# facebookresearch/sam-audio

Hardware: AMD Instinct MI355X
Metric: seconds-of-audio separated/sec/node (higher is better)
Workload: dtype fp16x3 (fp32 storage as the reference; every big contraction on IEEE-half hi + lo split operands: 3 MFMA products per multiply, fp32 accumulation - fp32-grade results on the 16-bit matrix cores)

## Files before the change

### sam_audio_amd/csrc/api.hip

```cpp
#include <cstring>
#include <string>

#include "engine.h"
#include "peav.h"

struct samaudio_ctx {
  sa::Engine* engine;
};
struct samaudio_judge {
  sa::Judge* judge;
};
struct samaudio_frame {
  sa::FramePredictor* frame;
};

namespace {
thread_local std::string g_err;
}
namespace sa {
void set_last_error(const std::string& msg) { g_err = msg; }
}
namespace {
int ret(const sa::Status& s) {
  if (!s.ok()) g_err = s.msg;
// ... 153 lines not shown
    out[n].ms = k.ms;
    ++n;
  }
  *count = n;
  return SAMAUDIO_OK;
}

int samaudio_op_gemm(const void* params_host, size_t params_bytes, int precision, samaudio_stream stream) {
  if (!params_host || params_bytes != sizeof(sa::GemmParams)) return bad("samaudio_op_gemm: GemmParams size mismatch");
  sa::GemmParams p;
  std::memcpy(&p, params_host, sizeof(p));
  const bool bf16 = precision == SAMAUDIO_BF16;
  if (const char* why = sa::gemm_check(p, bf16)) return bad(why);
  return hip_ret(sa::launch_gemm(p, bf16, (hipStream_t)stream), "gemm");
}

int samaudio_op_resunit(const void* conv7_params_host, const void* conv1_params_host, size_t params_bytes,
                        samaudio_stream stream) {
  if (!conv7_params_host || !conv1_params_host || params_bytes != sizeof(sa::GemmParams))
    return bad("samaudio_op_resunit: GemmParams size mismatch");
  sa::GemmParams p, q;
  std::memcpy(&p, conv7_params_host, sizeof(p));
  std::memcpy(&q, conv1_params_host, sizeof(q));
  if (const char* why = sa::gemm_check(p, true)) return bad(why);
  if (const char* why = sa::gemm_check(q, true)) return bad(why);
  if (!sa::resunit_ok(p, q)) return bad("samaudio_op_resunit: not a (k7, k1) residual-unit pair the fused kernel covers");
  return hip_ret(sa::launch_resunit(p, q, (hipStream_t)stream), "resunit");
}

int samaudio_op_rmsnorm_mod(const float* x, const float* w, const float* shift_tab, const float* scale_tab,
                            const float* tvec, int64_t tvec_ld, int shift_off, int scale_off, void* out,
                            int precision, int rows, int dim, int rows_per_batch, float eps, samaudio_stream stream) {
  if (dim % 4) return bad("rmsnorm_mod: dim % 4");
  return hip_ret(sa::launch_rmsnorm_mod(x, w, shift_tab, scale_tab, tvec, tvec_ld, shift_off, scale_off, out,
                                        precision == SAMAUDIO_BF16, rows, dim, rows_per_batch, eps,
                                        (hipStream_t)stream), "rmsnorm_mod");
}

int samaudio_op_groupnorm_silu(const float* x, const float* w, const float* b, void* partials_f64, void* out,
                               int precision, int batch, int frames, int channels, int halo, float eps,
                               samaudio_stream stream) {
  if (channels % 4) return bad("groupnorm: channels % 4");
  return hip_ret(sa::launch_groupnorm_silu(x, w, b, (double*)partials_f64, out, precision == SAMAUDIO_BF16, batch,
                                           frames, channels, halo, eps, (hipStream_t)stream), "groupnorm_silu");
}

int samaudio_op_qkv_prep(const void* qkv, const float* q_w, const float* k_w, const float* rope_cos,
                         const float* rope_sin, void* q, void* k, void* vt, int precision, int batch, int frames,
// ... 262 lines not shown
```

### sam_audio_amd/csrc/engine.hip

```cpp
#include "engine.h"

#include <algorithm>
#include <cmath>
#include <cstdio>
#include <cstdlib>
#include <cstring>

namespace sa {

#define SA_TRY(expr)                     \
  do {                                   \
    Status _s = (expr);                  \
    if (!_s.ok()) return _s;             \
  } while (0)
#define SA_HIP(expr)                                                                  \
  do {                                                                                \
    hipError_t _e = (expr);                                                           \
    if (_e != hipSuccess)                                                             \
      return Status{SAMAUDIO_ERR_HIP, std::string(#expr) + ": " + hipGetErrorString(_e)}; \
  } while (0)

static Status fail(int code, const std::string& m) { return Status{code, m}; }

static bool trace_on() {
// ... 752 lines not shown
  p.out_act = nullptr; p.act_ld = p.act_bstride = p.act_off = 0; p.act = ACT_NONE; p.f32_act = 0;
  const double flops = alg_flops >= 0 ? alg_flops : 2.0 * p_in.M * (double)p_in.N * p_in.K * p_in.nbatch;
  SA_TRY(gemm(p, st, flops, SAMAUDIO_CLS_CODEC, p_in.K == c && p_in.kc == c ? GemmKind::X3 : GemmKind::X3Block));
  if (!p_in.out_act || (act == ACT_NONE && !p_in.out_f32)) return Status{};
  const long start = p_in.c_ld_rel ? p_in.c_lo : 0, count = p_in.c_ld_rel ? p_in.c_hi - p_in.c_lo : (long)p_in.M * p_in.N;
  const int chan = p_in.chan_mod ? p_in.chan_mod : p_in.N;
  if (start % chan) return fail(SAMAUDIO_ERR_ARG, "gemm_codec_x3: window start is not a whole channel row");
  return op("codec_act", (double)count * p_in.nbatch * 8, 0, st, [&] {
    return launch_act_flat(raw + raw_off + start, raw_bs, (float*)p_in.out_act + p_in.act_off + start, p_in.act_bstride, p_in.nbatch, count,
                           chan, act, p_in.act_alpha, st);
  });
}

Status Engine::res_unit(GemmParams p, GemmParams q, void*& cur, void*& alt, double flops7, double flops1, hipStream_t st) {
  p.out_act = alt;
  q.A = alt;
  q.out_act = cur;
  GemmParams fp = p, fq = q;
  fq.out_act = alt;
  fp.tag = fq.tag = phase_ == Phase::Codec ? 1 : 0;
  const bool covered = p.N == 64 || p.N == 96 || p.N == 128 || p.N == 192;
  const bool fuse = bf16_ && covered && !debug_flag(DBG_RESUNIT_TWO_LAUNCHES) && resunit_ok(fp, fq) &&
                    ((long)((p.M + 255) / 256) * p.nbatch >= 256 || debug_flag(DBG_RESUNIT_FUSE_ALWAYS));
  if (!fuse) {
    SA_TRY(codec_gemm(p, st, flops7));
    return codec_gemm(q, st, flops1);
  }
  if (const char* why = gemm_check(fp, bf16_)) return fail(SAMAUDIO_ERR_ARG, why);
  if (const char* why = gemm_check(fq, bf16_)) return fail(SAMAUDIO_ERR_ARG, why);
  const double inter = (double)p.M * p.N * p.nbatch * esz_;
  SA_TRY(op("resunit_bf16", gemm_alg_bytes(fp, esz_) + gemm_alg_bytes(fq, esz_) - 2 * inter, flops7 + flops1, st,
            [&] { return launch_resunit(fp, fq, st); }));
  SA_TRY(scan_out(fq, SAMAUDIO_CLS_CODEC, GemmKind::Native, st));
  std::swap(cur, alt);
  return Status{};
}

template <class F>
Status Engine::op(const char* name, double alg_bytes, double alg_flops, hipStream_t st, F&& launch) {
  if (!prof_on_) {
    SA_HIP(launch());
    return Status{};
  }
  ProfRec r;
  r.key = std::string(phase_name()) + "/" + name;
  r.flops = alg_flops;
// ... 759 lines not shown
```

### sam_audio_amd/csrc/gemm.hip

```cpp
#include "common.h"
#include "kernels.h"

#include <type_traits>

namespace sa {

typedef h16x8_t bf16x8_t;
typedef __attribute__((ext_vector_type(4))) float f32x4_t;

template <typename T> struct Mma;
template <> struct Mma<bf16_t> {
  typedef bf16x8_t frag_t;
  static __device__ __forceinline__ f32x4_t run(const frag_t& a, const frag_t& b, f32x4_t c) {
    return SA_MFMA_16x16x32(a, b, c);
  }
};
template <> struct Mma<float> {
  typedef f32x4_t frag_t;
  static __device__ __forceinline__ f32x4_t run(const frag_t& a, const frag_t& b, f32x4_t c) {
    c = __builtin_amdgcn_mfma_f32_16x16x4f32(a[0], b[0], c, 0, 0, 0);
    c = __builtin_amdgcn_mfma_f32_16x16x4f32(a[1], b[1], c, 0, 0, 0);
    c = __builtin_amdgcn_mfma_f32_16x16x4f32(a[2], b[2], c, 0, 0, 0);
    c = __builtin_amdgcn_mfma_f32_16x16x4f32(a[3], b[3], c, 0, 0, 0);
    return c;
  }
};

__device__ __forceinline__ float quant16(float x, int fmt) {
  if (fmt == GEMM_QUANT_BF16) {
    unsigned u = __float_as_uint(x);
    u += 0x7fffu + ((u >> 16) & 1u);
    return __uint_as_float(u & 0xffff0000u);
  }
  if (fmt == GEMM_QUANT_FP16) return (float)(_Float16)x;
  return x;
}
__device__ __forceinline__ f32x4_t quant16x4(f32x4_t v, int fmt) {
  return f32x4_t{quant16(v[0], fmt), quant16(v[1], fmt), quant16(v[2], fmt), quant16(v[3], fmt)};
}

__device__ __forceinline__ void dma16(const void* gsrc, char* lds_wave_base) {
  __builtin_amdgcn_global_load_lds((const __attribute__((address_space(1))) void*)gsrc,
                                   (__attribute__((address_space(3))) void*)lds_wave_base, 16, 0, 0);
}

template <typename T, int BM, int BN, int WM_, int WN_, bool FLY = false>
__global__ __launch_bounds__(256, (FLY ? 2 : 1)) void gemm_kernel(const GemmParams p) {
  constexpr int NW = WM_ * WN_;
  static_assert(NW == 4, "4 waves per workgroup");
  constexpr int CH = 16 / (int)sizeof(T);
  constexpr int BK = 128 / (int)sizeof(T);
  constexpr int WTM = BM / WM_, WTN = BN / WN_;
  constexpr int FM = WTM / 16, FN = WTN / 16;
  constexpr int AI = BM / 32, BI = BN / 32;
  static_assert(BM % 32 == 0 && BN % 32 == 0 && WTM % 16 == 0 && WTN % 16 == 0, "tile shape");
  constexpr int TILE_A = BM * 128, TILE_B = BN * 128, STAGE = TILE_A + TILE_B;
  constexpr int NS = 2;
  __shared__ __attribute__((aligned(16))) char smem[NS * STAGE];

  const int tid = threadIdx.x;
  const int lane = tid & 63;
  const int wave = __builtin_amdgcn_readfirstlane(tid >> 6);
  const int wm = wave / WN_, wn = wave % WN_;

  const int tiles_n = (p.N + BN - 1) / BN;
  const int tiles_m = (p.M + BM - 1) / BM;
  int id = blockIdx.x;
  const int tn = id % tiles_n;
  id /= tiles_n;
  const int tm = id % tiles_m;
// ... 28 lines not shown
    char* sA = smem + stage * STAGE;
    char* sB = sA + TILE_A;
#pragma unroll
    for (int i = 0; i < AI; ++i) dma16(a_rows[i] + a_tap + a_in, sA + (wave + 4 * i) * 1024);
#pragma unroll
    for (int i = 0; i < BI; ++i) dma16(w_rows[i], sB + (wave + 4 * i) * 1024);
    a_in += BK;
    while (a_in >= p.kc) { a_in -= p.kc; a_tap += p.tap_stride; }
#pragma unroll
    for (int i = 0; i < BI; ++i) w_rows[i] += BK;
  };

  f32x4_t acc[FM][FN];
#pragma unroll
  for (int i = 0; i < FM; ++i)
#pragma unroll
    for (int j = 0; j < FN; ++j) acc[i][j] = f32x4_t{0.f, 0.f, 0.f, 0.f};

  const int nslab = p.K / BK;
  const int lr = lane & 15, lg = lane >> 4;
  const int qa = gemm_quant_a(p.flags), qw = gemm_quant_w(p.flags);
  const bool x3fly = FLY || (sizeof(T) == 4 && (p.flags & GEMM_FLAG_X3_FLY) != 0);
  const bool wfly = FLY || (p.flags & GEMM_FLAG_W_FLY16) != 0;
  auto fly_slab = [&](const char* sA, const char* sB) {
#pragma clang fp contract(off)
        bf16x8_t ah[FM], al[FM], bh[FN], bl[FN];
        auto cl = [](float x) { return __builtin_amdgcn_fmed3f(x, -kH16Max, kH16Max); };
        auto split = [&](const char* base, int row, bf16x8_t& hi, bf16x8_t& lo) {
          const int sw = (row >> 1) & 7;
          const f32x4_t v0 = *(const f32x4_t*)(base + row * 128 + ((lg ^ sw) << 4));
          const f32x4_t v1 = *(const f32x4_t*)(base + row * 128 + (((4 + lg) ^ sw) << 4));
          unsigned h[4], l[4];
          h[0] = pack_h16x2(cl(v0[0]), cl(v0[1]));
          h[1] = pack_h16x2(cl(v0[2]), cl(v0[3]));
          h[2] = pack_h16x2(cl(v1[0]), cl(v1[1]));
          h[3] = pack_h16x2(cl(v1[2]), cl(v1[3]));
          l[0] = pack_h16x2(v0[0] - h16_lo(h[0]), v0[1] - h16_hi(h[0]));
          l[1] = pack_h16x2(v0[2] - h16_lo(h[1]), v0[3] - h16_hi(h[1]));
          l[2] = pack_h16x2(v1[0] - h16_lo(h[2]), v1[1] - h16_hi(h[2]));
          l[3] = pack_h16x2(v1[2] - h16_lo(h[3]), v1[3] - h16_hi(h[3]));
          typedef __attribute__((ext_vector_type(4))) unsigned u32x4_t;
          hi = __builtin_bit_cast(bf16x8_t, (u32x4_t){h[0], h[1], h[2], h[3]});
          lo = __builtin_bit_cast(bf16x8_t, (u32x4_t){l[0], l[1], l[2], l[3]});
        };
        if (wfly) {
#pragma unroll
          for (int j = 0; j < FN; ++j) {
            const int row = wn * WTN + j * 16 + lr, sw = (row >> 1) & 7;
            bh[j] = *(const bf16x8_t*)(sB + row * 128 + ((lg ^ sw) << 4));
            bl[j] = *(const bf16x8_t*)(sB + row * 128 + (((4 + lg) ^ sw) << 4));
          }
        } else {
#pragma unroll
          for (int j = 0; j < FN; ++j) split(sB, wn * WTN + j * 16 + lr, bh[j], bl[j]);
        }
#pragma unroll
        for (int i = 0; i < FM; ++i) split(sA, wm * WTM + i * 16 + lr, ah[i], al[i]);
#pragma unroll
        for (int i = 0; i < FM; ++i)
#pragma unroll
          for (int j = 0; j < FN; ++j) acc[i][j] = SA_MFMA_16x16x32(bh[j], al[i], acc[i][j]);
#pragma unroll
        for (int i = 0; i < FM; ++i)
#pragma unroll
          for (int j = 0; j < FN; ++j) acc[i][j] = SA_MFMA_16x16x32(bl[j], ah[i], acc[i][j]);
#pragma unroll
// ... 27 lines not shown
#pragma unroll
      for (int j = 0; j < FN; ++j) {
        const int row = wn * WTN + j * 16 + lr;
        bfr[j] = *(const typename Mma<T>::frag_t*)(sB + row * 128 + ((c ^ ((row >> 1) & 7)) << 4));
      }
      if constexpr (sizeof(T) == 4) {
        if (qa) {
#pragma unroll
          for (int i = 0; i < FM; ++i) af[i] = quant16x4(af[i], qa);
        }
        if (qw) {
#pragma unroll
          for (int j = 0; j < FN; ++j) bfr[j] = quant16x4(bfr[j], qw);
        }
      }
#pragma unroll
      for (int i = 0; i < FM; ++i)
#pragma unroll
        for (int j = 0; j < FN; ++j) acc[i][j] = Mma<T>::run(bfr[j], af[i], acc[i][j]);
    }
    }
  }

  const long bM = (long)b * p.M;
  const int n_out = p.swiglu ? p.N >> 1 : p.N;
  auto finish = [&](float v, const float bias, const float gate, const float res, const float sa, float& a) -> float {
    v += bias;
    if (p.gate) v *= gate;
    v *= p.alpha;
    v += res;
    a = v;
    if (p.act == ACT_SNAKE) a = snake_f(v, sa);
    else if (p.act == ACT_TANH) a = tanhf(v);
    else if (p.act == ACT_SILU) a = silu_f(v);
    else if (p.act == ACT_GELU) a = gelu_f(v);
    else if (p.act == ACT_QUICK_GELU) a = quick_gelu_f(v);
    else if (p.act == ACT_RELU) a = relu_f(v);
    else if (p.act == ACT_GELU_TANH) a = gelu_tanh_f(v);
    return v;
  };
  if constexpr (sizeof(T) == 4) {
    auto al16 = [](const void* q, long a, long b2, long c) { return (((size_t)q) & 15) == 0 && !((a | b2 | c) & 3); };
    const bool lean = !p.swiglu && !p.gate && !p.chan_mod && !p.c_ld_rel && !(p.N & 3) && (!p.bias || al16(p.bias, 0, 0, 0)) &&
                      (p.act != ACT_SNAKE || al16(p.act_alpha, 0, 0, 0)) && (!p.res || al16(p.res, p.res_off, p.res_ld, p.res_bstride)) &&
                      (!p.out_f32 || al16(p.out_f32, p.f32_off, p.f32_ld, p.f32_bstride)) &&
                      (!p.out_act || al16(p.out_act, p.act_off, p.act_ld, p.act_bstride));
    if (lean && (p.act == ACT_NONE || p.act == ACT_SNAKE)) {
      constexpr int CPR = BN / 4, RPI = 64 / CPR, WR = BM / 4, NIT = (WR + RPI - 1) / RPI;
      static_assert(BN % 32 == 0 && BM * BN * 4 <= NS * STAGE, "epilogue staging area");
      __syncthreads();
#pragma unroll
      for (int i = 0; i < FM; ++i)
#pragma unroll
        for (int j = 0; j < FN; ++j) {
          const int row = wm * WTM + i * 16 + lr, c = wn * (WTN / 4) + j * 4 + lg;
          *(f32x4_t*)(smem + row * (BN * 4) + ((c ^ (row & 7)) << 4)) = acc[i][j];
        }
      __syncthreads();
      const float4 z = make_float4(0.f, 0.f, 0.f, 0.f);
      const int c = lane % CPR, rsub = lane / CPR;
      const bool lane_on = rsub < RPI;
      const int n = n0 + c * 4;
      const int ncl = n < p.N ? n : p.N - 4;
      const float4 bb = p.bias ? *(const float4*)(p.bias + ncl) : z;
      const float4 sa = p.act == ACT_SNAKE ? *(const float4*)(p.act_alpha + ncl) : z;
      const float* const res0 = p.res ? p.res + p.res_off + (long)b * p.res_bstride + ncl : nullptr;
      float* const f320 = p.out_f32 ? p.out_f32 + p.f32_off + (long)b * p.f32_bstride + n : nullptr;
      float* const act0 = p.out_act ? (float*)p.out_act + p.act_off + (long)b * p.act_bstride + n : nullptr;
      const int rw = wave * WR;
      auto body = [&](auto SNAKE) {
        auto fin = [&](float v, const float bias, const float res, const float sal, float& a) -> float {
          v += bias;
          v *= p.alpha;
          v += res;
          a = decltype(SNAKE)::value ? snake_f(v, sal) : v;
          return v;
        };
        auto res_of = [&](int it) {
          const int m = m0 + rw + it * RPI + rsub;
          return res0 ? *(const float4*)(res0 + (long)(m < p.M ? m : p.M - 1) * p.res_ld) : z;
        };
        float4 rr = res_of(0);
#pragma unroll 1
        for (int it = 0; it < NIT; ++it) {
          const float4 rn = it + 1 < NIT ? res_of(it + 1) : z;
          const int rl = it * RPI + rsub, row = rw + (rl < WR ? rl : 0), m = m0 + row;
          const float4 sv = *(const float4*)(smem + row * (BN * 4) + ((c ^ (row & 7)) << 4));
          float a0, a1, a2, a3;
          const float v0 = fin(sv.x, bb.x, rr.x, sa.x, a0), v1 = fin(sv.y, bb.y, rr.y, sa.y, a1), v2 = fin(sv.z, bb.z, rr.z, sa.z, a2),
                      v3 = fin(sv.w, bb.w, rr.w, sa.w, a3);
          if (lane_on && rl < WR && m < p.M && n < p.N) {
            if (f320) *(float4*)(f320 + (long)m * p.f32_ld) = p.f32_act ? make_float4(a0, a1, a2, a3) : make_float4(v0, v1, v2, v3);
            if (act0) *(float4*)(act0 + (long)m * p.act_ld) = make_float4(a0, a1, a2, a3);
          }
          rr = rn;
        }
      };
      if (p.act == ACT_SNAKE) body(std::true_type{});
      else body(std::false_type{});
      return;
    }
  }
#pragma unroll
  for (int i = 0; i < FM; ++i) {
    const int m = m0 + wm * WTM + i * 16 + lr;
    if (m >= p.M) continue;
    const float* grow = nullptr;
    if (p.gate) grow = p.gate + ((bM + m) / p.rows_per_gate) * p.gate_ld;
    const float* rrow = p.res ? p.res + p.res_off + (long)b * p.res_bstride + (long)m * p.res_ld : nullptr;
    float* frow = p.out_f32 ? p.out_f32 + p.f32_off + (long)b * p.f32_bstride + (long)m * p.f32_ld : nullptr;
    T* arow = p.out_act ? (T*)p.out_act + p.act_off + (long)b * p.act_bstride + (long)m * p.act_ld : nullptr;
#pragma unroll
    for (int j = 0; j < FN; ++j) {
      if (p.swiglu && (j & 1)) continue;
      f32x4_t v4 = acc[i][j];
      int n = n0 + wn * WTN + j * 16 + lg * 4;
      if (p.swiglu) {
        const f32x4_t g = acc[i][j | 1];
#pragma unroll
        for (int e = 0; e < 4; ++e) v4[e] = silu_f(v4[e]) * g[e];
        n = ((n0 + wn * WTN) >> 1) + (j >> 1) * 16 + lg * 4;
      }
      if (n >= n_out) continue;
      size_t al = 0;
      if (p.bias) al |= (size_t)(p.bias + n);
      if (grow) al |= (size_t)(grow + n);
      if (p.gate_tab) al |= (size_t)(p.gate_tab + n);
      if (rrow) al |= (size_t)(rrow + n);
      if (p.act == ACT_SNAKE) al |= (size_t)(p.act_alpha + n);
      if (frow) al |= (size_t)(frow + n);
      if (arow) al |= (size_t)(arow + n) * (16 / (4 * sizeof(T)));
      if (n + 4 <= n_out && !p.chan_mod && !p.c_ld_rel && (al & 15) == 0) {
        const float4 z = make_float4(0.f, 0.f, 0.f, 0.f);
        const float4 bb = p.bias ? *(const float4*)(p.bias + n) : z;
        float4 gg = grow ? *(const float4*)(grow + n) : z;
        if (grow && p.gate_tab) { const float4 tt = *(const float4*)(p.gate_tab + n); gg.x += tt.x; gg.y += tt.y; gg.z += tt.z; gg.w += tt.w; }
        const float4 rr = rrow ? *(const float4*)(rrow + n) : z;
        const float4 sa = p.act == ACT_SNAKE ? *(const float4*)(p.act_alpha + n) : z;
        float a0, a1, a2, a3;
        const float v0 = finish(v4[0], bb.x, gg.x, rr.x, sa.x, a0), v1 = finish(v4[1], bb.y, gg.y, rr.y, sa.y, a1),
                    v2 = finish(v4[2], bb.z, gg.z, rr.z, sa.z, a2), v3 = finish(v4[3], bb.w, gg.w, rr.w, sa.w, a3);
        if (frow) *(float4*)(frow + n) = p.f32_act ? make_float4(a0, a1, a2, a3) : make_float4(v0, v1, v2, v3);
        if (arow) store4<T>(arow + n, a0, a1, a2, a3);
        continue;
      }
#pragma unroll
      for (int e = 0; e < 4; ++e) {
        const int ne = n + e;
        if (ne >= n_out) continue;
        const int ch = p.chan_mod ? ne % p.chan_mod : ne;
        const long erel = (long)m * p.c_ld_rel + ne;
        if (p.c_ld_rel && (erel < p.c_lo || erel >= p.c_hi)) continue;
        float a;
        const float v = finish(v4[e], p.bias ? p.bias[ch] : 0.f, grow ? (p.gate_tab ? p.gate_tab[ne] : 0.f) + grow[ne] : 0.f,
                               rrow ? rrow[ne] : 0.f, p.act == ACT_SNAKE ? p.act_alpha[ch] : 0.f, a);
        if (frow) frow[ne] = p.f32_act ? a : v;
        if (arow) Elem<T>::store(arow + ne, a);
      }
    }
  }
}

template <typename T, int BM, int BN, int WM_, int WN_>
static hipError_t launch_cfg(const GemmParams& p, hipStream_t st) {
  const long tiles = (long)((p.M + BM - 1) / BM) * ((p.N + BN - 1) / BN) * p.nbatch;
  hipLaunchKernelGGL((gemm_kernel<T, BM, BN, WM_, WN_>), dim3((unsigned)tiles), dim3(256), 0, st, p);
  return hipGetLastError();
}

static int g_force = -1;
void gemm_force_variant(int v) { g_force = v; }

const char* gemm_variant_name(int v, bool is_bf16) {
  const GemmVariantRow* r = gemm_variant_row(v);
  return !r ? "" : is_bf16 ? r->name16 : r->name32;
}

static GemmVariant gemm1_variant(const GemmParams& p) {
  const int N = p.N;
  if (p.swiglu) return GV_GEMM_128x128;
  if (N <= 32 || N == 96) return GV_GEMM_128x32;
  if (N <= 64 || (N % 128 != 0 && N % 64 == 0 && N <= 448)) return GV_GEMM_128x64;
  const long t128 = (long)((p.M + 127) / 128) * ((N + 127) / 128) * p.nbatch;
// ... 54 lines not shown
}

hipError_t launch_gemm(const GemmParams& p, bool is_bf16, hipStream_t st) {
  if (const int full = gemm_tail_split(p, is_bf16)) {
    const hipError_t e = launch_gemm8_split(p, full, 0, st);
    return e != hipSuccess ? e : launch_gemm8_split(p, full, 1, st);
  }
  const int v = gemm_variant(p, is_bf16);
  if (v >= GV_FLY_128x96) {
    const auto go = [&](auto kern, int bm, int bn) {
      const long tiles = (long)((p.M + bm - 1) / bm) * ((p.N + bn - 1) / bn) * p.nbatch;
      hipLaunchKernelGGL(kern, dim3((unsigned)tiles), dim3(256), 0, st, p);
      return hipGetLastError();
    };
    switch (v) {
      case GV_FLY_128x96: return go(gemm_kernel<float, 128, 96, 4, 1, true>, 128, 96);
      case GV_FLY_128x128: return go(gemm_kernel<float, 128, 128, 4, 1, true>, 128, 128);
      case GV_FLY_128x64: return go(gemm_kernel<float, 128, 64, 4, 1, true>, 128, 64);
      default: return go(gemm_kernel<float, 128, 32, 4, 1, true>, 128, 32);
    }
  }
  if (v > GV_GEMM_128x32) return launch_gemm2(p, (GemmVariant)v, st);
  return is_bf16 ? launch_t<bf16_t>(p, v, st) : launch_t<float>(p, v, st);
}

static const char* need_8phase(const GemmParams& p, bool is_bf16, bool (*eligible)(const GemmParams&), const char* not_eligible,
                               const char* not_chosen) {
  if (!is_bf16 || !gemm2_ok(p) || !eligible(p)) return not_eligible;
  return gemm_is_8phase(gemm_variant(p, is_bf16)) ? nullptr : not_chosen;
}
const char* gemm_check(const GemmParams& p, bool is_bf16) {
  const int bk = is_bf16 ? 64 : 32, ch = is_bf16 ? 8 : 4;
  if (p.M <= 0 || p.N <= 0 || p.K <= 0 || p.nbatch <= 0) return "gemm: empty problem";
  if (p.K % bk) return "gemm: K must be a multiple of 64 (bf16) / 32 (f32) - pad W with zeros";
  if (p.kc % ch || p.kc <= 0) return "gemm: kc must be a positive multiple of the 16-byte chunk";
  if ((p.lda % ch) || (p.tap_stride % ch) || (p.a_off % ch) || (p.a_bstride % ch))
    return "gemm: A strides/offsets must be 16-byte aligned";
  if (p.swiglu && (p.N % 32)) return "gemm: swiglu needs N % 32 == 0";
  if (p.gate && p.rows_per_gate <= 0) return "gemm: rows_per_gate";
  if ((p.flags & GEMM_FLAG_W_FLY16) && (is_bf16 || !(p.flags & GEMM_FLAG_X3_FLY)))
    return "gemm: split-weight layout (flags bit 14): fp32 launches with operands split on the fly (bit 13) only";
  if (p.flags & (GEMM_FLAG_OUT_ALT | GEMM_FLAG_OPND_ALT))
    if (const char* e = need_8phase(p, is_bf16, gemm8_alt_ok, "gemm: alt 16-bit format: plain 16-bit launches with a lean epilogue only",
                                    "gemm: alt 16-bit format: the tile policy did not pick the 8-phase family for this launch")) return e;
  if (p.flags & GEMM_FLAG_OUT_SPLIT3)
    if (const char* e = need_8phase(p, is_bf16, gemm8_split3_ok, "gemm: split3 output: 16-bit SwiGLU launches with a lean epilogue only",
// ... 13 lines not shown
```

### sam_audio_amd/csrc/gemm2.hip

```cpp
#include "common.h"
#include "kernels.h"

namespace sa {

typedef h16x8_t bf16x8_t;
typedef __attribute__((ext_vector_type(16))) float f32x16_t;
typedef __attribute__((ext_vector_type(4))) float f32x4_t;

namespace {

__device__ __forceinline__ void dma16(const void* gsrc, char* lds_wave_base) {
  __builtin_amdgcn_global_load_lds((const __attribute__((address_space(1))) void*)gsrc,
                                   (__attribute__((address_space(3))) void*)lds_wave_base, 16, 0, 0);
}
__device__ __forceinline__ void dma16a(const void* gsrc, char* lds_wave_base) {
  const unsigned lds = __builtin_amdgcn_readfirstlane((unsigned)(size_t)(__attribute__((address_space(3))) char*)lds_wave_base);
  asm volatile("s_mov_b32 m0, %0\n\ts_nop 0\n\tglobal_load_lds_dwordx4 %1, off" ::"s"(lds), "v"(gsrc) : "memory", "m0");
}

template <int N> __device__ __forceinline__ void wait_vmcnt() {
  asm volatile("s_waitcnt vmcnt(%0)" ::"n"(N) : "memory");
}
__device__ __forceinline__ float act_apply(float v, int act, float snake_alpha) {
  if (act == ACT_SILU) return silu_f(v);
// ... 706 lines not shown
}

template <int C, int BM, int WM_, int WN_, int STAGES>
static hipError_t launch_c7(const GemmParams& p, hipStream_t st) {
  const long tiles = (long)((p.M + BM - 1) / BM) * p.nbatch;
  if (p.tag == 1)
    hipLaunchKernelGGL((conv7h_kernel<C, BM, WM_, WN_, STAGES, 1>), dim3((unsigned)tiles), dim3(512), 0, st, p);
  else
    hipLaunchKernelGGL((conv7h_kernel<C, BM, WM_, WN_, STAGES, 0>), dim3((unsigned)tiles), dim3(512), 0, st, p);
  return hipGetLastError();
}

hipError_t launch_conv7h(const GemmParams& p, hipStream_t st) {
  switch (p.N) {
    case 64: return launch_c7<64, 256, 8, 1, 3>(p, st);
    case 96: return launch_c7<96, 256, 8, 1, 3>(p, st);
    case 128: return launch_c7<128, 256, 4, 2, 3>(p, st);
    case 192: return launch_c7<192, 128, 4, 2, 3>(p, st);
    default: return hipErrorInvalidValue;
  }
}

bool resunit_ok(const GemmParams& p, const GemmParams& q) {
  if (!conv7h_ok(p) || !gemm2_ok(q)) return false;
  if (q.N != p.N || q.M != p.M || q.nbatch != p.nbatch || q.kc != p.N || q.lda != p.N || q.w_bstride != 0) return false;
  if (q.K != (p.N + 63) / 64 * 64 || q.swiglu || q.gate || q.chan_mod || q.c_ld_rel || q.alpha != 1.f) return false;
  if (p.gate || p.chan_mod || p.c_ld_rel || p.res || p.out_f32 || p.f32_act || !p.out_act) return false;
  if (p.act != ACT_SNAKE && p.act != ACT_NONE) return false;
  if (q.A != p.out_act || q.a_off != p.act_off || q.a_bstride != p.act_bstride || p.act_ld != p.N) return false;
  if (!q.out_act || q.out_act == p.A) return false;
  return true;
}

template <int C, int BM, int WM_, int WN_, int STAGES>
static hipError_t launch_ru(const GemmParams& p, const GemmParams& q, hipStream_t st) {
  const long tiles = (long)((p.M + BM - 1) / BM) * p.nbatch;
  if (p.tag == 1)
    hipLaunchKernelGGL((resunit_kernel<C, BM, WM_, WN_, STAGES, 1>), dim3((unsigned)tiles), dim3(WM_ * WN_ * 64), 0, st, p, q);
  else
    hipLaunchKernelGGL((resunit_kernel<C, BM, WM_, WN_, STAGES, 0>), dim3((unsigned)tiles), dim3(WM_ * WN_ * 64), 0, st, p, q);
  return hipGetLastError();
}

template <int C>
static hipError_t launch_ws(const GemmParams& p, const GemmParams& q, long tiles, hipStream_t st) {
  const long cap = debug_flag(DBG_RESUNIT_WS) == DBG_WS_ALWAYS_GRID3 ? 3 : 256;
  const unsigned grid = (unsigned)(tiles < cap ? tiles : cap);
  if (p.tag == 1)
    hipLaunchKernelGGL((resws_kernel<C, 1>), dim3(grid), dim3(C / 32 * 64), 0, st, p, q);
  else
    hipLaunchKernelGGL((resws_kernel<C, 0>), dim3(grid), dim3(C / 32 * 64), 0, st, p, q);
  return hipGetLastError();
}

static bool resunit_ws(const GemmParams& p, const GemmParams& q) {
  if (!(p.N == 64 || p.N == 96) || debug_flag(DBG_RESUNIT_WS) == DBG_WS_NEVER) return false;
  if (q.act != ACT_SNAKE && q.act != ACT_NONE) return false;
  if (debug_flag(DBG_RESUNIT_WS) == DBG_WS_ALWAYS || debug_flag(DBG_RESUNIT_WS) == DBG_WS_ALWAYS_GRID3) return true;
  return p.N == 96 && (long)((p.M + 127) / 128) * p.nbatch >= 1024;
}

hipError_t launch_resunit(const GemmParams& p, const GemmParams& q, hipStream_t st) {
  if (resunit_ws(p, q)) {
    const long tiles = (long)((p.M + 127) / 128) * p.nbatch;
    return p.N == 64 ? launch_ws<64>(p, q, tiles, st) : launch_ws<96>(p, q, tiles, st);
  }
  switch (p.N) {
    case 64: return launch_ru<64, 256, 8, 1, 3>(p, q, st);
    case 96: return launch_ru<96, 128, 4, 1, 2>(p, q, st);
    case 128: return launch_ru<128, 256, 4, 2, 3>(p, q, st);
    case 192: return launch_ru<192, 128, 4, 2, 3>(p, q, st);
    default: return hipErrorInvalidValue;
  }
}

template <int BM, int BN, int WM_, int WN_, int STAGES, int BK, bool TAGGED = false>
static hipError_t launch2(const GemmParams& p, hipStream_t st) {
  const long tiles = (long)((p.M + BM - 1) / BM) * ((p.N + BN - 1) / BN) * p.nbatch;
  if (TAGGED && p.tag == 1)
    hipLaunchKernelGGL((gemm2_kernel<BM, BN, WM_, WN_, STAGES, BK, TAGGED ? 1 : 0>), dim3((unsigned)tiles),
                       dim3(WM_ * WN_ * 64), 0, st, p);
  else
    hipLaunchKernelGGL((gemm2_kernel<BM, BN, WM_, WN_, STAGES, BK, 0>), dim3((unsigned)tiles), dim3(WM_ * WN_ * 64), 0,
                       st, p);
  return hipGetLastError();
// ... 37 lines not shown
```

### sam_audio_amd/csrc/kernels.h

```cpp
#pragma once
#include "common.h"

namespace sa {

hipError_t launch_poison_lds(hipStream_t st);

enum DebugFlag : int {
  DBG_NO_CONV7H = 11,
  DBG_RESUNIT_TWO_LAUNCHES = 16,
  DBG_RESUNIT_FUSE_ALWAYS = 18,
  DBG_RESUNIT_WS = 19,
  DBG_GEMM8S_PLAIN = 21,
  DBG_GEMM8_EPILOGUE = 24,
  DBG_GEMM8_NOT_PERSISTENT = 26,
  DBG_GEMM8S_ROLES = 27,
  DBG_QKV_PREP_SWROUND = 29,
  DBG_GEMM8_MIN_TILES = 30,
  DBG_FOLD_PER_LAYER = 31,
  DBG_TAIL_SPLIT_MIN = 33,
  DBG_RASTER_GM = 35,
  DBG_FLY_OLD_TILES = 36,
  DBG_X3_PLAIN_WALK = 38,
};
enum : int { DBG_WS_ALWAYS = 1, DBG_WS_NEVER = 2, DBG_WS_ALWAYS_GRID3 = 3 };
// ... 55 lines not shown
    {GV_FLY_128x64, FAM_FLY, "", "gemm_f32x3_128x64"},
    {GV_FLY_128x32, FAM_FLY, "", "gemm_f32x3_128x32"},
};
constexpr const GemmVariantRow* gemm_variant_row(int v) {
  for (const GemmVariantRow& r : kGemmVariantTable)
    if (r.id == v) return &r;
  return nullptr;
}
constexpr bool gemm_is_8phase(int v) { return gemm_variant_row(v) && gemm_variant_row(v)->family == FAM_8PHASE; }
constexpr const char* kGemm8sTailName = "gemm8s_bf16_128x128_tail";
int gemm_variant(const GemmParams& p, bool is_bf16);
const char* gemm_variant_name(int variant, bool is_bf16);
bool gemm2_ok(const GemmParams& p);
hipError_t launch_gemm2(const GemmParams& p, GemmVariant variant, hipStream_t st);
hipError_t launch_gemm8(const GemmParams& p, hipStream_t st);
bool gemm8_share_ok(const GemmParams& p);
hipError_t launch_gemm8s(const GemmParams& p, hipStream_t st);
bool gemm8_alt_ok(const GemmParams& p);
bool gemm8_split3_ok(const GemmParams& p);
bool conv7h_ok(const GemmParams& p);
hipError_t launch_conv7h(const GemmParams& p, hipStream_t st);
bool resunit_ok(const GemmParams& p, const GemmParams& q);
hipError_t launch_resunit(const GemmParams& p, const GemmParams& q, hipStream_t st);
hipError_t launch_gemm8_split(const GemmParams& p, int full, int part, hipStream_t st);
int gemm_tail_split(const GemmParams& p, bool is_bf16);
hipError_t launch_gemm_part(const GemmParams& p, bool is_bf16, int part, hipStream_t st);
void gemm_force_variant(int v);

hipError_t launch_rmsnorm_mod(const float* x, const float* w, const float* shift_tab, const float* scale_tab,
                              const float* tvec, long tvec_ld, int shift_off, int scale_off, void* out, bool bf16,
                              int M, int D, int rows_per_b, float eps, hipStream_t st);

hipError_t launch_layernorm_accum(const float* x, const float* w, const float* b, const float* gate, float* acc,
                                  int M, int D, float eps, hipStream_t st);

hipError_t launch_groupnorm_silu(const float* x, const float* w, const float* b, double* partials, void* out,
                                 bool bf16, int B, int T, int C, int halo, float eps, hipStream_t st);

constexpr int kMaxModNorms = 96;
struct ModTables {
  const float* w[kMaxModNorms];
  const float* shift_tab[kMaxModNorms];
  const float* scale_tab[kMaxModNorms];
  int shift_off[kMaxModNorms], scale_off[kMaxModNorms];
};
hipError_t launch_mod_tables(const ModTables& t, int n_norms, const float* tvec, long tvec_ld, int nt, float* gs, int D,
// ... 109 lines not shown
```

Measured before the change: 94.86.

## Fuse codec residual unit k7+k1 convs into one fp16x3 fly kernel

Adds a fused residual-unit path for fp16x3 (X3_FLY) codec convolutions. The k7 conv's snake-activated output tile stays in registers, is split into hi/lo halves and multiplied by the k1 weights in the same kernel, so the intermediate activation is never written to and re-read from global memory and one launch is saved. The shared gemm body is templated with an RU mode, and its lean epilogue is extended to windowed outputs. The change raises register pressure, holds full-width N tiles per wave, and is skipped for N=192 by default.

Result: no change. 95.53, median of 6 (+0.7%).

```diff
diff --git a/profiles/resunit_x3/unit_bench.py b/profiles/resunit_x3/unit_bench.py
--- /dev/null
+++ b/profiles/resunit_x3/unit_bench.py
@@ -0,0 +1,39 @@
+import ctypes as CT, math, sys, torch
+sys.path.insert(0, ".")
+from sam_audio_amd import hip
+from sam_audio_amd.weights import fly16_weight
+from tests import util
+gpu = torch.device("cuda:0")
+lib = hip.lib("fp16")
+FLY = hip.GEMM_FLAG_X3_FLY | hip.GEMM_FLAG_W_FLY16
+HALO = 40
+def run(C, T, items, dil=3, iters=10):
+    g = torch.Generator().manual_seed(1)
+    xin = torch.zeros(items, T + 2 * HALO, C, device=gpu); xin[:, HALO:HALO + T] = torch.randn(items, T, C, device=gpu)
+    W7 = fly16_weight(torch.randn(C, 7 * C, generator=g) / math.sqrt(7 * C), torch.float16).to(gpu)
+    W1 = fly16_weight(torch.randn(C, C, generator=g) / math.sqrt(C), torch.float16).to(gpu)
+    b7, a7, b1, a1 = [(torch.rand(C, generator=g) + 0.5).to(gpu) for _ in range(4)]
+    mid = torch.zeros_like(xin); out = torch.zeros_like(xin); raw = torch.zeros_like(xin)
+    geom = ((T + 2 * HALO) * C, C, HALO * C)
+    p7 = util.gemm_params(xin, W7, T, C, 7 * C, nbatch=items, a_off=(HALO - 3 * dil) * C, a_bstride=geom[0], lda=C, kc=C, tap_stride=dil * C,
+                          bias=b7, out_act=mid, act_geom=geom, act=hip.ACT_SNAKE, act_alpha=a7, flags=FLY)
+    p1 = util.gemm_params(mid, W1, T, C, C, nbatch=items, a_off=HALO * C, a_bstride=geom[0], lda=C, kc=C, tap_stride=C, bias=b1, res=raw,
+                          res_geom=geom, out_f32=raw, f32_geom=geom, out_act=out, act_geom=geom, act=hip.ACT_SNAKE, act_alpha=a1, flags=FLY)
+    def two():
+        for p in (p7, p1):
+            hip.check(lib.samaudio_op_gemm(CT.byref(p), CT.sizeof(p), hip.F32, util.stream()))
+    def k7():
+        hip.check(lib.samaudio_op_gemm(CT.byref(p7), CT.sizeof(p7), hip.F32, util.stream()))
+    def fused():
+        util.resunit(p7, p1, "fp16x3")
+    res = {}
+    for name, fn in (("two", two), ("k7 alone", k7), ("fused", fused), ("two", two), ("fused", fused)):
+        fn(); torch.cuda.synchronize()
+        e0, e1 = torch.cuda.Event(enable_timing=True), torch.cuda.Event(enable_timing=True)
+        e0.record()
+        for _ in range(iters): fn()
+        e1.record(); torch.cuda.synchronize()
+        res.setdefault(name, []).append(e0.elapsed_time(e1) / iters)
+    print(f"C={C} rows={T * items}: " + "; ".join(f"{k} {' / '.join(f'{v:.3f}' for v in vs)} ms" for k, vs in res.items()), flush=True)
+for C, T, items in ((64, 240000, 8), (96, 240000, 8), (96, 120000, 8), (128, 120000, 8), (192, 120000, 8), (192, 60000, 8)):
+    run(C, T, items)
diff --git a/sam_audio_amd/csrc/api.hip b/sam_audio_amd/csrc/api.hip
--- a/sam_audio_amd/csrc/api.hip
+++ b/sam_audio_amd/csrc/api.hip
@@ -199,8 +199,9 @@
   sa::GemmParams p, q;
   std::memcpy(&p, conv7_params_host, sizeof(p));
   std::memcpy(&q, conv1_params_host, sizeof(q));
-  if (const char* why = sa::gemm_check(p, true)) return bad(why);
-  if (const char* why = sa::gemm_check(q, true)) return bad(why);
+  const bool bf16 = !((p.flags | q.flags) & sa::GEMM_FLAG_X3_FLY);
+  if (const char* why = sa::gemm_check(p, bf16)) return bad(why);
+  if (const char* why = sa::gemm_check(q, bf16)) return bad(why);
   if (!sa::resunit_ok(p, q)) return bad("samaudio_op_resunit: not a (k7, k1) residual-unit pair the fused kernel covers");
   return hip_ret(sa::launch_resunit(p, q, (hipStream_t)stream), "resunit");
 }
diff --git a/sam_audio_amd/csrc/engine.hip b/sam_audio_amd/csrc/engine.hip
--- a/sam_audio_amd/csrc/engine.hip
+++ b/sam_audio_amd/csrc/engine.hip
@@ -798,6 +798,30 @@
   const bool covered = p.N == 64 || p.N == 96 || p.N == 128 || p.N == 192;
   const bool fuse = bf16_ && covered && !debug_flag(DBG_RESUNIT_TWO_LAUNCHES) && resunit_ok(fp, fq) &&
                     ((long)((p.M + 255) / 256) * p.nbatch >= 256 || debug_flag(DBG_RESUNIT_FUSE_ALWAYS));
+  if (!fuse && x3(SAMAUDIO_CLS_CODEC) && !debug_flag(DBG_RESUNIT_TWO_LAUNCHES) && !codec_x3_twin(p) && !codec_x3_twin(q) &&
+      (p.N != 192 || debug_flag(DBG_RESUNIT_FUSE_ALWAYS))) {
+    GemmParams* const both[2] = {&fp, &fq};
+    bool twins = true;
+    for (GemmParams* g : both) {
+      *g = launch_params(*g, SAMAUDIO_CLS_CODEC, GemmKind::Native);
+      const auto it = g->w_bstride ? fly_codec_.end() : fly_codec_.find(g->W);
+      if (it == fly_codec_.end()) { twins = false; break; }
+      g->W = it->second;
+      g->flags |= GEMM_FLAG_X3_FLY | GEMM_FLAG_W_FLY16;
+    }
+    if (twins && resunit_ok(fp, fq)) {
+      if (const char* why = gemm_check(fp, false)) return fail(SAMAUDIO_ERR_ARG, why);
+      if (const char* why = gemm_check(fq, false)) return fail(SAMAUDIO_ERR_ARG, why);
+      const double inter = (double)p.M * p.N * p.nbatch * 4;
+      SA_TRY(op("resunit_f32x3", gemm_alg_bytes(fp, 4) + gemm_alg_bytes(fq, 4) - 2 * inter, flops7 + flops1, st,
+                [&] { return launch_resunit(fp, fq, st); }));
+      GemmParams out = q;
+      out.out_act = alt;
+      SA_TRY(scan_out(out, SAMAUDIO_CLS_CODEC, GemmKind::Native, st));
+      std::swap(cur, alt);
+      return Status{};
+    }
+  }
   if (!fuse) {
     SA_TRY(codec_gemm(p, st, flops7));
     return codec_gemm(q, st, flops1);
diff --git a/sam_audio_amd/csrc/gemm.hip b/sam_audio_amd/csrc/gemm.hip
--- a/sam_audio_amd/csrc/gemm.hip
+++ b/sam_audio_amd/csrc/gemm.hip
@@ -44,8 +44,8 @@
                                    (__attribute__((address_space(3))) void*)lds_wave_base, 16, 0, 0);
 }
 
-template <typename T, int BM, int BN, int WM_, int WN_, bool FLY = false>
-__global__ __launch_bounds__(256, (FLY ? 2 : 1)) void gemm_kernel(const GemmParams p) {
+template <typename T, int BM, int BN, int WM_, int WN_, bool FLY, bool RU>
+__device__ __forceinline__ void gemm_body(const GemmParams& p, const GemmParams& q) {
   constexpr int NW = WM_ * WN_;
   static_assert(NW == 4, "4 waves per workgroup");
   constexpr int CH = 16 / (int)sizeof(T);
@@ -120,14 +120,9 @@
   const int qa = gemm_quant_a(p.flags), qw = gemm_quant_w(p.flags);
   const bool x3fly = FLY || (sizeof(T) == 4 && (p.flags & GEMM_FLAG_X3_FLY) != 0);
   const bool wfly = FLY || (p.flags & GEMM_FLAG_W_FLY16) != 0;
-  auto fly_slab = [&](const char* sA, const char* sB) {
+  auto split_vals = [](const f32x4_t v0, const f32x4_t v1, bf16x8_t& hi, bf16x8_t& lo) {
 #pragma clang fp contract(off)
-        bf16x8_t ah[FM], al[FM], bh[FN], bl[FN];
-        auto cl = [](float x) { return __builtin_amdgcn_fmed3f(x, -kH16Max, kH16Max); };
-        auto split = [&](const char* base, int row, bf16x8_t& hi, bf16x8_t& lo) {
-          const int sw = (row >> 1) & 7;
-          const f32x4_t v0 = *(const f32x4_t*)(base + row * 128 + ((lg ^ sw) << 4));
-          const f32x4_t v1 = *(const f32x4_t*)(base + row * 128 + (((4 + lg) ^ sw) << 4));
+          auto cl = [](float x) { return __builtin_amdgcn_fmed3f(x, -kH16Max, kH16Max); };
           unsigned h[4], l[4];
           h[0] = pack_h16x2(cl(v0[0]), cl(v0[1]));
           h[1] = pack_h16x2(cl(v0[2]), cl(v0[3]));
@@ -140,6 +135,12 @@
           typedef __attribute__((ext_vector_type(4))) unsigned u32x4_t;
           hi = __builtin_bit_cast(bf16x8_t, (u32x4_t){h[0], h[1], h[2], h[3]});
           lo = __builtin_bit_cast(bf16x8_t, (u32x4_t){l[0], l[1], l[2], l[3]});
+  };
+  auto fly_slab = [&](const char* sA, const char* sB) {
+        bf16x8_t ah[FM], al[FM], bh[FN], bl[FN];
+        auto split = [&](const char* base, int row, bf16x8_t& hi, bf16x8_t& lo) {
+          const int sw = (row >> 1) & 7;
+          split_vals(*(const f32x4_t*)(base + row * 128 + ((lg ^ sw) << 4)), *(const f32x4_t*)(base + row * 128 + (((4 + lg) ^ sw) << 4)), hi, lo);
         };
         if (wfly) {
 #pragma unroll
@@ -213,30 +214,84 @@
     }
   }
 
-  const long bM = (long)b * p.M;
-  const int n_out = p.swiglu ? p.N >> 1 : p.N;
+  if constexpr (RU) {
+    static_assert(FLY && WN_ == 1 && FN % 2 == 0, "fused residual unit: full-width FLY tiles");
+    constexpr int NSL = FN / 2;
+    const f32x4_t z4 = f32x4_t{0.f, 0.f, 0.f, 0.f};
+    bf16x8_t xh[FM][NSL], xl[FM][NSL];
+#pragma unroll
+    for (int i = 0; i < FM; ++i) {
+#pragma unroll
+      for (int j = 0; j < FN; ++j) {
+        const int n = j * 16 + lg * 4;
+        const f32x4_t bb = p.bias ? *(const f32x4_t*)(p.bias + n) : z4;
+        const f32x4_t sa = p.act == ACT_SNAKE ? *(const f32x4_t*)(p.act_alpha + n) : z4;
+#pragma unroll
+        for (int e = 0; e < 4; ++e) {
+          float v = acc[i][j][e];
+          v += bb[e];
+          v *= p.alpha;
+          v += 0.f;
+          acc[i][j][e] = p.act == ACT_SNAKE ? snake_f(v, sa[e]) : v;
+        }
+      }
+#pragma unroll
+      for (int s = 0; s < NSL; ++s) split_vals(acc[i][2 * s], acc[i][2 * s + 1], xh[i][s], xl[i][s]);
+#pragma unroll
+      for (int j = 0; j < FN; ++j) acc[i][j] = z4;
+    }
+    const char* const w1 = (const char*)q.W + (long)lr * q.K * 4 + (lg << 4);
+#pragma unroll
+    for (int s = 0; s < NSL; ++s) {
+      bf16x8_t bh[FN], bl[FN];
+#pragma unroll
+      for (int j = 0; j < FN; ++j) {
+        const char* const w = w1 + (long)j * 16 * q.K * 4 + s * 128;
+        bh[j] = *(const bf16x8_t*)w;
+        bl[j] = *(const bf16x8_t*)(w + 64);
+      }
+#pragma unroll
+      for (int i = 0; i < FM; ++i)
+#pragma unroll
+        for (int j = 0; j < FN; ++j) acc[i][j] = SA_MFMA_16x16x32(bh[j], xl[i][s], acc[i][j]);
+#pragma unroll
+      for (int i = 0; i < FM; ++i)
+#pragma unroll
+        for (int j = 0; j < FN; ++j) acc[i][j] = SA_MFMA_16x16x32(bl[j], xh[i][s], acc[i][j]);
+#pragma unroll
+      for (int i = 0; i < FM; ++i)
+#pragma unroll
+        for (int j = 0; j < FN; ++j) acc[i][j] = SA_MFMA_16x16x32(bh[j], xh[i][s], acc[i][j]);
+    }
+  }
+
+  const GemmParams& ep = RU ? q : p;
+  const long bM = (long)b * ep.M;
+  const int n_out = ep.swiglu ? ep.N >> 1 : ep.N;
   auto finish = [&](float v, const float bias, const float gate, const float res, const float sa, float& a) -> float {
     v += bias;
-    if (p.gate) v *= gate;
-    v *= p.alpha;
+    if (ep.gate) v *= gate;
+    v *= ep.alpha;
     v += res;
     a = v;
-    if (p.act == ACT_SNAKE) a = snake_f(v, sa);
-    else if (p.act == ACT_TANH) a = tanhf(v);
-    else if (p.act == ACT_SILU) a = silu_f(v);
-    else if (p.act == ACT_GELU) a = gelu_f(v);
-    else if (p.act == ACT_QUICK_GELU) a = quick_gelu_f(v);
-    else if (p.act == ACT_RELU) a = relu_f(v);
-    else if (p.act == ACT_GELU_TANH) a = gelu_tanh_f(v);
+    if (ep.act == ACT_SNAKE) a = snake_f(v, sa);
+    else if (ep.act == ACT_TANH) a = tanhf(v);
+    else if (ep.act == ACT_SILU) a = silu_f(v);
+    else if (ep.act == ACT_GELU) a = gelu_f(v);
+    else if (ep.act == ACT_QUICK_GELU) a = quick_gelu_f(v);
+    else if (ep.act == ACT_RELU) a = relu_f(v);
+    else if (ep.act == ACT_GELU_TANH) a = gelu_tanh_f(v);
     return v;
   };
   if constexpr (sizeof(T) == 4) {
     auto al16 = [](const void* q, long a, long b2, long c) { return (((size_t)q) & 15) == 0 && !((a | b2 | c) & 3); };
-    const bool lean = !p.swiglu && !p.gate && !p.chan_mod && !p.c_ld_rel && !(p.N & 3) && (!p.bias || al16(p.bias, 0, 0, 0)) &&
-                      (p.act != ACT_SNAKE || al16(p.act_alpha, 0, 0, 0)) && (!p.res || al16(p.res, p.res_off, p.res_ld, p.res_bstride)) &&
-                      (!p.out_f32 || al16(p.out_f32, p.f32_off, p.f32_ld, p.f32_bstride)) &&
-                      (!p.out_act || al16(p.out_act, p.act_off, p.act_ld, p.act_bstride));
-    if (lean && (p.act == ACT_NONE || p.act == ACT_SNAKE)) {
+    const bool win = ep.chan_mod || ep.c_ld_rel;
+    const bool win_ok = FLY && !((ep.chan_mod | ep.c_ld_rel | ep.c_lo | ep.c_hi) & 3);
+    const bool lean = !ep.swiglu && !ep.gate && (!win || win_ok) && !(ep.N & 3) && (!ep.bias || al16(ep.bias, 0, 0, 0)) &&
+                      (ep.act != ACT_SNAKE || al16(ep.act_alpha, 0, 0, 0)) && (!ep.res || al16(ep.res, ep.res_off, ep.res_ld, ep.res_bstride)) &&
+                      (!ep.out_f32 || al16(ep.out_f32, ep.f32_off, ep.f32_ld, ep.f32_bstride)) &&
+                      (!ep.out_act || al16(ep.out_act, ep.act_off, ep.act_ld, ep.act_bstride));
+    if (lean && (ep.act == ACT_NONE || ep.act == ACT_SNAKE)) {
       constexpr int CPR = BN / 4, RPI = 64 / CPR, WR = BM / 4, NIT = (WR + RPI - 1) / RPI;
       static_assert(BN % 32 == 0 && BM * BN * 4 <= NS * STAGE, "epilogue staging area");
       __syncthreads();
@@ -252,24 +307,25 @@
       const int c = lane % CPR, rsub = lane / CPR;
       const bool lane_on = rsub < RPI;
       const int n = n0 + c * 4;
-      const int ncl = n < p.N ? n : p.N - 4;
-      const float4 bb = p.bias ? *(const float4*)(p.bias + ncl) : z;
-      const float4 sa = p.act == ACT_SNAKE ? *(const float4*)(p.act_alpha + ncl) : z;
-      const float* const res0 = p.res ? p.res + p.res_off + (long)b * p.res_bstride + ncl : nullptr;
-      float* const f320 = p.out_f32 ? p.out_f32 + p.f32_off + (long)b * p.f32_bstride + n : nullptr;
-      float* const act0 = p.out_act ? (float*)p.out_act + p.act_off + (long)b * p.act_bstride + n : nullptr;
+      const int ncl = n < ep.N ? n : ep.N - 4;
+      const int nch = ep.chan_mod ? ncl % ep.chan_mod : ncl;
+      const float4 bb = ep.bias ? *(const float4*)(ep.bias + nch) : z;
+      const float4 sa = ep.act == ACT_SNAKE ? *(const float4*)(ep.act_alpha + nch) : z;
+      const float* const res0 = ep.res ? ep.res + ep.res_off + (long)b * ep.res_bstride + ncl : nullptr;
+      float* const f320 = ep.out_f32 ? ep.out_f32 + ep.f32_off + (long)b * ep.f32_bstride + n : nullptr;
+      float* const act0 = ep.out_act ? (float*)ep.out_act + ep.act_off + (long)b * ep.act_bstride + n : nullptr;
       const int rw = wave * WR;
       auto body = [&](auto SNAKE) {
         auto fin = [&](float v, const float bias, const float res, const float sal, float& a) -> float {
           v += bias;
-          v *= p.alpha;
+          v *= ep.alpha;
           v += res;
           a = decltype(SNAKE)::value ? snake_f(v, sal) : v;
           return v;
         };
         auto res_of = [&](int it) {
           const int m = m0 + rw + it * RPI + rsub;
-          return res0 ? *(const float4*)(res0 + (long)(m < p.M ? m : p.M - 1) * p.res_ld) : z;
+          return res0 ? *(const float4*)(res0 + (long)(m < ep.M ? m : ep.M - 1) * ep.res_ld) : z;
         };
         float4 rr = res_of(0);
 #pragma unroll 1
@@ -280,33 +336,35 @@
           float a0, a1, a2, a3;
           const float v0 = fin(sv.x, bb.x, rr.x, sa.x, a0), v1 = fin(sv.y, bb.y, rr.y, sa.y, a1), v2 = fin(sv.z, bb.z, rr.z, sa.z, a2),
                       v3 = fin(sv.w, bb.w, rr.w, sa.w, a3);
-          if (lane_on && rl < WR && m < p.M && n < p.N) {
-            if (f320) *(float4*)(f320 + (long)m * p.f32_ld) = p.f32_act ? make_float4(a0, a1, a2, a3) : make_float4(v0, v1, v2, v3);
-            if (act0) *(float4*)(act0 + (long)m * p.act_ld) = make_float4(a0, a1, a2, a3);
+          const long erel = (long)m * ep.c_ld_rel + n;
+          if (lane_on && rl < WR && m < ep.M && n < ep.N && (!ep.c_ld_rel || (erel >= ep.c_lo && erel < ep.c_hi))) {
+            if (f320) *(float4*)(f320 + (long)m * ep.f32_ld) = ep.f32_act ? make_float4(a0, a1, a2, a3) : make_float4(v0, v1, v2, v3);
+            if (act0) *(float4*)(act0 + (long)m * ep.act_ld) = make_float4(a0, a1, a2, a3);
           }
           rr = rn;
         }
       };
-      if (p.act == ACT_SNAKE) body(std::true_type{});
+      if (ep.act == ACT_SNAKE) body(std::true_type{});
       else body(std::false_type{});
       return;
     }
   }
+  if constexpr (RU) return;
 #pragma unroll
   for (int i = 0; i < FM; ++i) {
     const int m = m0 + wm * WTM + i * 16 + lr;
-    if (m >= p.M) continue;
+    if (m >= ep.M) continue;
     const float* grow = nullptr;
-    if (p.gate) grow = p.gate + ((bM + m) / p.rows_per_gate) * p.gate_ld;
-    const float* rrow = p.res ? p.res + p.res_off + (long)b * p.res_bstride + (long)m * p.res_ld : nullptr;
-    float* frow = p.out_f32 ? p.out_f32 + p.f32_off + (long)b * p.f32_bstride + (long)m * p.f32_ld : nullptr;
-    T* arow = p.out_act ? (T*)p.out_act + p.act_off + (long)b * p.act_bstride + (long)m * p.act_ld : nullptr;
+    if (ep.gate) grow = ep.gate + ((bM + m) / ep.rows_per_gate) * ep.gate_ld;
+    const float* rrow = ep.res ? ep.res + ep.res_off + (long)b * ep.res_bstride + (long)m * ep.res_ld : nullptr;
+    float* frow = ep.out_f32 ? ep.out_f32 + ep.f32_off + (long)b * ep.f32_bstride + (long)m * ep.f32_ld : nullptr;
+    T* arow = ep.out_act ? (T*)ep.out_act + ep.act_off + (long)b * ep.act_bstride + (long)m * ep.act_ld : nullptr;
 #pragma unroll
     for (int j = 0; j < FN; ++j) {
-      if (p.swiglu && (j & 1)) continue;
+      if (ep.swiglu && (j & 1)) continue;
       f32x4_t v4 = acc[i][j];
       int n = n0 + wn * WTN + j * 16 + lg * 4;
-      if (p.swiglu) {
+      if (ep.swiglu) {
         const f32x4_t g = acc[i][j | 1];
 #pragma unroll
         for (int e = 0; e < 4; ++e) v4[e] = silu_f(v4[e]) * g[e];
@@ -314,24 +372,24 @@
       }
       if (n >= n_out) continue;
       size_t al = 0;
-      if (p.bias) al |= (size_t)(p.bias + n);
+      if (ep.bias) al |= (size_t)(ep.bias + n);
       if (grow) al |= (size_t)(grow + n);
-      if (p.gate_tab) al |= (size_t)(p.gate_tab + n);
+      if (ep.gate_tab) al |= (size_t)(ep.gate_tab + n);
       if (rrow) al |= (size_t)(rrow + n);
-      if (p.act == ACT_SNAKE) al |= (size_t)(p.act_alpha + n);
+      if (ep.act == ACT_SNAKE) al |= (size_t)(ep.act_alpha + n);
       if (frow) al |= (size_t)(frow + n);
       if (arow) al |= (size_t)(arow + n) * (16 / (4 * sizeof(T)));
-      if (n + 4 <= n_out && !p.chan_mod && !p.c_ld_rel && (al & 15) == 0) {
+      if (n + 4 <= n_out && !ep.chan_mod && !ep.c_ld_rel && (al & 15) == 0) {
         const float4 z = make_float4(0.f, 0.f, 0.f, 0.f);
-        const float4 bb = p.bias ? *(const float4*)(p.bias + n) : z;
+        const float4 bb = ep.bias ? *(const float4*)(ep.bias + n) : z;
         float4 gg = grow ? *(const float4*)(grow + n) : z;
-        if (grow && p.gate_tab) { const float4 tt = *(const float4*)(p.gate_tab + n); gg.x += tt.x; gg.y += tt.y; gg.z += tt.z; gg.w += tt.w; }
+        if (grow && ep.gate_tab) { const float4 tt = *(const float4*)(ep.gate_tab + n); gg.x += tt.x; gg.y += tt.y; gg.z += tt.z; gg.w += tt.w; }
         const float4 rr = rrow ? *(const float4*)(rrow + n) : z;
-        const float4 sa = p.act == ACT_SNAKE ? *(const float4*)(p.act_alpha + n) : z;
+        const float4 sa = ep.act == ACT_SNAKE ? *(const float4*)(ep.act_alpha + n) : z;
         float a0, a1, a2, a3;
         const float v0 = finish(v4[0], bb.x, gg.x, rr.x, sa.x, a0), v1 = finish(v4[1], bb.y, gg.y, rr.y, sa.y, a1),
                     v2 = finish(v4[2], bb.z, gg.z, rr.z, sa.z, a2), v3 = finish(v4[3], bb.w, gg.w, rr.w, sa.w, a3);
-        if (frow) *(float4*)(frow + n) = p.f32_act ? make_float4(a0, a1, a2, a3) : make_float4(v0, v1, v2, v3);
+        if (frow) *(float4*)(frow + n) = ep.f32_act ? make_float4(a0, a1, a2, a3) : make_float4(v0, v1, v2, v3);
         if (arow) store4<T>(arow + n, a0, a1, a2, a3);
         continue;
       }
@@ -339,17 +397,26 @@
       for (int e = 0; e < 4; ++e) {
         const int ne = n + e;
         if (ne >= n_out) continue;
-        const int ch = p.chan_mod ? ne % p.chan_mod : ne;
-        const long erel = (long)m * p.c_ld_rel + ne;
-        if (p.c_ld_rel && (erel < p.c_lo || erel >= p.c_hi)) continue;
+        const int ch = ep.chan_mod ? ne % ep.chan_mod : ne;
+        const long erel = (long)m * ep.c_ld_rel + ne;
+        if (ep.c_ld_rel && (erel < ep.c_lo || erel >= ep.c_hi)) continue;
         float a;
-        const float v = finish(v4[e], p.bias ? p.bias[ch] : 0.f, grow ? (p.gate_tab ? p.gate_tab[ne] : 0.f) + grow[ne] : 0.f,
-                               rrow ? rrow[ne] : 0.f, p.act == ACT_SNAKE ? p.act_alpha[ch] : 0.f, a);
-        if (frow) frow[ne] = p.f32_act ? a : v;
+        const float v = finish(v4[e], ep.bias ? ep.bias[ch] : 0.f, grow ? (ep.gate_tab ? ep.gate_tab[ne] : 0.f) + grow[ne] : 0.f,
+                               rrow ? rrow[ne] : 0.f, ep.act == ACT_SNAKE ? ep.act_alpha[ch] : 0.f, a);
+        if (frow) frow[ne] = ep.f32_act ? a : v;
         if (arow) Elem<T>::store(arow + ne, a);
       }
     }
   }
+}
+
+template <typename T, int BM, int BN, int WM_, int WN_, bool FLY = false>
+__global__ __launch_bounds__(256, (FLY ? 2 : 1)) void gemm_kernel(const GemmParams p) {
+  gemm_body<T, BM, BN, WM_, WN_, FLY, false>(p, p);
+}
+template <int BM, int BN>
+__global__ __launch_bounds__(256, 2) void gemm_kernel_resunit(const GemmParams p, const GemmParams q) {
+  gemm_body<float, BM, BN, 4, 1, true, true>(p, q);
 }
 
 template <typename T, int BM, int BN, int WM_, int WN_>
@@ -450,6 +517,37 @@
   }
   if (v > GV_GEMM_128x32) return launch_gemm2(p, (GemmVariant)v, st);
   return is_bf16 ? launch_t<bf16_t>(p, v, st) : launch_t<float>(p, v, st);
+}
+
+static bool fly_lean_ok(const GemmParams& p) {
+  const auto al = [](const void* ptr, long a, long b, long c) { return (((size_t)ptr) & 15) == 0 && !((a | b | c) & 3); };
+  return !p.swiglu && !p.gate && !p.chan_mod && !p.c_ld_rel && !(p.N & 3) && (!p.bias || al(p.bias, 0, 0, 0)) &&
+         (p.act == ACT_NONE || (p.act == ACT_SNAKE && p.act_alpha && al(p.act_alpha, 0, 0, 0))) &&
+         (!p.res || al(p.res, p.res_off, p.res_ld, p.res_bstride)) && (!p.out_f32 || al(p.out_f32, p.f32_off, p.f32_ld, p.f32_bstride)) &&
+         (!p.out_act || al(p.out_act, p.act_off, p.act_ld, p.act_bstride));
+}
+bool resunit_fly_ok(const GemmParams& p, const GemmParams& q) {
+  constexpr int fly = GEMM_FLAG_X3_FLY | GEMM_FLAG_W_FLY16;
+  if ((p.flags & fly) != fly || (q.flags & fly) != fly || p.w_bstride || q.w_bstride) return false;
+  if (!(p.N == 64 || p.N == 96 || p.N == 128 || p.N == 192) || q.N != p.N || q.K != p.N || q.kc != p.N || q.lda != p.N) return false;
+  if (q.M != p.M || q.nbatch != p.nbatch) return false;
+  if (!fly_lean_ok(p) || p.res || p.out_f32 || p.f32_act || !p.out_act) return false;
+  if (!fly_lean_ok(q) || !q.out_act || q.out_act == p.A) return false;
+  return q.A == p.out_act && q.a_off == p.act_off && q.a_bstride == p.act_bstride && p.act_ld == p.N;
+}
+hipError_t launch_resunit_fly(const GemmParams& p, const GemmParams& q, hipStream_t st) {
+  const auto go = [&](auto kern, int bm) {
+    const long tiles = (long)((p.M + bm - 1) / bm) * p.nbatch;
+    hipLaunchKernelGGL(kern, dim3((unsigned)tiles), dim3(256), 0, st, p, q);
+    return hipGetLastError();
+  };
+  switch (p.N) {
+    case 64: return go(gemm_kernel_resunit<128, 64>, 128);
+    case 96: return go(gemm_kernel_resunit<128, 96>, 128);
+    case 128: return go(gemm_kernel_resunit<128, 128>, 128);
+    case 192: return go(gemm_kernel_resunit<64, 192>, 64);
+    default: return hipErrorInvalidValue;
+  }
 }
 
 static const char* need_8phase(const GemmParams& p, bool is_bf16, bool (*eligible)(const GemmParams&), const char* not_eligible,
diff --git a/sam_audio_amd/csrc/gemm2.hip b/sam_audio_amd/csrc/gemm2.hip
--- a/sam_audio_amd/csrc/gemm2.hip
+++ b/sam_audio_amd/csrc/gemm2.hip
@@ -752,6 +752,7 @@
 }
 
 bool resunit_ok(const GemmParams& p, const GemmParams& q) {
+  if ((p.flags | q.flags) & GEMM_FLAG_X3_FLY) return resunit_fly_ok(p, q);
   if (!conv7h_ok(p) || !gemm2_ok(q)) return false;
   if (q.N != p.N || q.M != p.M || q.nbatch != p.nbatch || q.kc != p.N || q.lda != p.N || q.w_bstride != 0) return false;
   if (q.K != (p.N + 63) / 64 * 64 || q.swiglu || q.gate || q.chan_mod || q.c_ld_rel || q.alpha != 1.f) return false;
@@ -791,6 +792,7 @@
 }
 
 hipError_t launch_resunit(const GemmParams& p, const GemmParams& q, hipStream_t st) {
+  if (p.flags & GEMM_FLAG_X3_FLY) return launch_resunit_fly(p, q, st);
   if (resunit_ws(p, q)) {
     const long tiles = (long)((p.M + 127) / 128) * p.nbatch;
     return p.N == 64 ? launch_ws<64>(p, q, tiles, st) : launch_ws<96>(p, q, tiles, st);
diff --git a/sam_audio_amd/csrc/kernels.h b/sam_audio_amd/csrc/kernels.h
--- a/sam_audio_amd/csrc/kernels.h
+++ b/sam_audio_amd/csrc/kernels.h
@@ -101,6 +101,8 @@
 hipError_t launch_conv7h(const GemmParams& p, hipStream_t st);
 bool resunit_ok(const GemmParams& p, const GemmParams& q);
 hipError_t launch_resunit(const GemmParams& p, const GemmParams& q, hipStream_t st);
+bool resunit_fly_ok(const GemmParams& p, const GemmParams& q);
+hipError_t launch_resunit_fly(const GemmParams& p, const GemmParams& q, hipStream_t st);
 hipError_t launch_gemm8_split(const GemmParams& p, int full, int part, hipStream_t st);
 int gemm_tail_split(const GemmParams& p, bool is_bf16);
 hipError_t launch_gemm_part(const GemmParams& p, bool is_bf16, int part, hipStream_t st);
```
